# Charrrrrlie/X-as-Supervision

Measured on AMD Instinct MI355X. Metric: images/sec HM36_Multi_SurS1 256px bs32 (full disc+gen training step), higher is better.
Workload: dtype f32 (f16x3 split: every fp32 operand as two fp16 pieces, three products; f32 accumulate); 1 GPU; HM36_Multi_SurS1; batch_per_gpu=32, cameras=4, image=256x256, parallelism=dp1, ranks=1, precision=f16x3, dedupe=False, full=False

## Files before the change

### include/xas_hip.h

```cpp
#ifndef XAS_HIP_H
#define XAS_HIP_H

#include <stddef.h>
#include <stdint.h>

#ifdef __cplusplus
extern "C" {
#endif

const char* xas_last_error(void);
enum {
  XAS_TUNE_WGRAD_SPLIT_XCD = 1,
  XAS_TUNE_PLAIN_KLOOP = 32,
  XAS_TUNE_GLOBAL_LOAD = 64,
  XAS_TUNE_WGRAD_GLOBAL_LOAD = 128,
  XAS_TUNE_WGRAD_ALT_ORDER = 8192,
  XAS_TUNE_WGRAD_PLAIN_KLOOP = 524288,
  XAS_TUNE_SLAB_SHIFT = 15,
  XAS_TUNE_SLAB_MASK = 3,
  XAS_TUNE_SLAB_512 = 32768,
  XAS_TUNE_SLAB_128 = 65536,
  XAS_TUNE_SLAB_64 = 98304,
  XAS_TUNE_COL_REDUCE_LEAN = 262144,
  XAS_TUNE_GENERAL_KERNELS = 1 << 22,
// ... 139 lines not shown
                      const float* var_biased, const float* gamma, const float* beta, float eps, int act,
                      long M, int C, int groups, float* sums, float* workspace,
                      float* dbeta_acc, float* dgamma_acc, const uint8_t* mask, void* stream);
int xas_bn_bwd_apply(const float* x, const float* y, const float* dy, const float* mean,
                     const float* var_biased, const float* gamma, const float* beta, const float* sums,
                     float eps, int act, long M, int C, int groups, double count,
                     float* dx, float* dresidual, const uint8_t* mask, void* stream);
int xas_bn_bwd_apply_amax(const float* x, const float* y, const float* dy, const float* mean,
                          const float* var_biased, const float* gamma, const float* beta, const float* sums,
                          float eps, int act, long M, int C, int groups, double count, float* dx,
                          float* dresidual, const uint8_t* mask, float* amax_out, void* stream);

int xas_maxpool3x3s2_fwd(const float* x, int N, int H, int W, int C, float* y, int8_t* idx, void* stream);
int xas_maxpool3x3s2_bwd(const float* dy, const int8_t* idx, int N, int H, int W, int C, float* dx, void* stream);

int xas_upsample2x_fwd(const float* x, int N, int H, int W, int C, float* y, void* stream);
int xas_upsample2x_bwd(const float* dy, int N, int H, int W, int C, float* dx, void* stream);

int xas_sigmoid_fwd(const float* x, long n, float* y, void* stream);
int xas_sigmoid_bwd(const float* y, const float* dy, long n, float* dx, void* stream);
int xas_nchw_to_nhwc(const float* x, int N, int C, int H, int W, float* y, void* stream);
int xas_nhwc_to_nchw(const float* x, int N, int C, int H, int W, float* y, void* stream);

int xas_warp_affine_u8(const uint8_t* src, const long* src_off, const int* src_hw, const double* minv, int B, int C,
                       int P, uint8_t* dst, void* stream);
int xas_mask_blur_threshold(const uint8_t* mask, int B, int P, uint8_t* out, void* stream);
int xas_patch_finish(const uint8_t* img_bgr, const uint8_t* mask, const float* color_scale, const float* mean3,
                     const float* std3, int rm_bg, int B, int P, float* out_img, float* out_mask, void* stream);
size_t xas_geodesic_workspace_bytes(int B, int P);
int xas_geodesic_weight(const float* mask, const int* centers, const float* params5, int B, int P, float* out,
// ... 73 lines not shown
```

### x-as-supervision_amd/csrc/bn.hip

```cpp
#include "common.h"

namespace xas {


struct ColGeom { int TX, TY, CB, ncb, nslab, G; long rows_per_slab, Mg; };

static int col_geom(long M, int C, int G, ColGeom* g) {
  XAS_REQUIRE(M > 0 && C >= 4 && C % 4 == 0, "column reduce: channel count %d must be a positive multiple of 4", C);
  XAS_REQUIRE(G >= 1 && G <= 64 && M % G == 0, "column reduce: %ld rows do not split into %d equal groups", M, G);
  int cb = 4;
  while (cb < 64 && C % (cb * 2) == 0) cb *= 2;
  g->CB = cb; g->G = G; g->Mg = M / G;
  g->TX = g->CB / 4; g->TY = 256 / g->TX; g->ncb = C / g->CB;
  static const long kWant[4] = {256, 512, 128, 64};
  long want = kWant[(tune_flags() >> XAS_TUNE_SLAB_SHIFT) & XAS_TUNE_SLAB_MASK] * (G > 1 ? 2 : 1) / ((long)g->ncb * G);
  long maxslab = cdiv(g->Mg, (long)g->TY * 8);
  if (want > maxslab) want = maxslab;
  if (want < 1) want = 1;
  g->rows_per_slab = cdiv(g->Mg, want);
  g->nslab = (int)cdiv(g->Mg, g->rows_per_slab);
  return 0;
}

constexpr int kTicketWords = 65536;
// ... 19 lines not shown
  unsafeAtomicAdd(p + 0, v.x); unsafeAtomicAdd(p + 1, v.y); unsafeAtomicAdd(p + 2, v.z); unsafeAtomicAdd(p + 3, v.w);
}

#ifndef XAS_BN_PRIO
#define XAS_BN_PRIO 3
#endif

enum ColMode : int {
  kColStats = 0,
  kColBwdXY = 1,
  kColSum = 2,
  kColBwdY = 3,
  kColBwdX = 4,
  kColStatsPartials = 5,
  kColBwdPartials = 6,
};
constexpr bool col_is_bwd(ColMode m) { return m == kColBwdXY || m == kColBwdY || m == kColBwdX; }
constexpr bool col_two_sums(ColMode m) { return m == kColStats || col_is_bwd(m); }
constexpr bool col_is_stats(ColMode m) { return m == kColStats || m == kColStatsPartials; }

struct ColArgs {
  const float* x; const float* y; const float* dy;
  const float* mean; const float* var;
  const float* gamma; const float* beta;
  const float* pivot;
  const uint8_t* mask;
  float eps; int act; long M; int C; ColGeom g;
  float* partial;
  unsigned* ticket;
  float* out1; float* out2;
  long out_stride;
  float* count_out;
  float* running_mean; float* running_var; float momentum, unbias;
  float* acc1; float* acc2;
  long rows_real;
};

// ... 21 lines not shown
  return dz;
}
__device__ __forceinline__ float4 dz_sign_mask(float4 dz, unsigned mb, float neg) {
  dz.x *= (mb & 1u) ? 1.f : neg; dz.y *= (mb & 2u) ? 1.f : neg; dz.z *= (mb & 4u) ? 1.f : neg; dz.w *= (mb & 8u) ? 1.f : neg;
  return dz;
}
__device__ __forceinline__ float4 xhat4(float4 v, const float4& m, const float4& s) {
  return make_float4((v.x - m.x) * s.x, (v.y - m.y) * s.y, (v.z - m.z) * s.z, (v.w - m.w) * s.w);
}
__device__ __forceinline__ float4 act_inv4(float4 yv, int act) {
  const float up = act == 1 ? 0.f : 100.f;
  return make_float4(yv.x > 0.f ? yv.x : yv.x * up, yv.y > 0.f ? yv.y : yv.y * up, yv.z > 0.f ? yv.z : yv.z * up,
                     yv.w > 0.f ? yv.w : yv.w * up);
}

struct ColChan {
  float4 pivot, mean, rstd, rsg, beta, inv_gamma;
};

template <ColMode MODE>
__device__ __forceinline__ ColChan col_chan(const ColArgs& a, int grp, int c) {
  ColChan ch{};
  if constexpr (MODE == kColStats) ch.pivot = ld4(a.x + (size_t)grp * a.g.Mg * a.C + c);
  if constexpr (MODE == kColBwdXY || MODE == kColBwdX) {
    ch.mean = ld4(a.mean + (size_t)grp * a.C + c);
    const float4 v = ld4(a.var + (size_t)grp * a.C + c);
    ch.rstd = make_float4(rsqrtf(v.x + a.eps), rsqrtf(v.y + a.eps), rsqrtf(v.z + a.eps), rsqrtf(v.w + a.eps));
  }
  if constexpr (MODE == kColBwdX) {
    const float4 gm = ld4(a.gamma + c);
    ch.rsg = make_float4(__fmul_rn(ch.rstd.x, gm.x), __fmul_rn(ch.rstd.y, gm.y), __fmul_rn(ch.rstd.z, gm.z), __fmul_rn(ch.rstd.w, gm.w));
    ch.beta = ld4(a.beta + c);
  }
  if constexpr (MODE == kColBwdY) {
    ch.beta = ld4(a.beta + c);
    const float4 gm = ld4(a.gamma + c);
    ch.inv_gamma = make_float4(gm.x != 0.f ? 1.f / gm.x : 0.f, gm.y != 0.f ? 1.f / gm.y : 0.f, gm.z != 0.f ? 1.f / gm.z : 0.f,
                               gm.w != 0.f ? 1.f / gm.w : 0.f);
  }
  return ch;
}

struct ColTerm { float4 f1, w; };

template <ColMode MODE>
__device__ __forceinline__ ColTerm col_term(const ColArgs& a, const ColChan& ch, long i) {
  const float neg = act_neg_slope(a.act);
  if constexpr (MODE == kColBwdY) {
    const float4 dz = ld4(a.dy + i), yv = ld4(a.y + i);
    return {dz_sign_y(dz, yv, neg), xhat4(act_inv4(yv, a.act), ch.beta, ch.inv_gamma)};
  } else {
    const float4 xv = ld4(a.x + i);
    if constexpr (MODE == kColStats) {
      const float4 d = make_float4(xv.x - ch.pivot.x, xv.y - ch.pivot.y, xv.z - ch.pivot.z, xv.w - ch.pivot.w);
      return {d, d};
    } else if constexpr (MODE == kColBwdXY) {
      float4 dz = ld4(a.dy + i);
      if (a.act && a.mask) dz = dz_sign_mask(dz, a.mask[i >> 2], neg);
      else if (a.act) dz = dz_sign_y(dz, ld4(a.y + i), neg);
      return {dz, xhat4(xv, ch.mean, ch.rstd)};
    } else if constexpr (MODE == kColBwdX) {
      return {dz_sign_x(ld4(a.dy + i), xv, ch.mean, ch.rsg, ch.beta, neg), xhat4(xv, ch.mean, ch.rstd)};
    } else {
      return {xv, xv};
    }
  }
}

__device__ __forceinline__ bool col_publish(const ColArgs& a, float4 (&red)[2][256], __amdgpu_buffer_rsrc_t prs, float4 s1,
                                            float4 s2, int tx, int ty, int c, int grp) {
  const ColGeom& g = a.g;
  red[0][threadIdx.x] = s1; red[1][threadIdx.x] = s2;
  __syncthreads();
  for (int s = g.TY >> 1; s > 0; s >>= 1) {
    if (ty < s) {
      const float4 u0 = red[0][threadIdx.x + s * g.TX], v0 = red[1][threadIdx.x + s * g.TX];
      float4& u = red[0][threadIdx.x]; float4& v = red[1][threadIdx.x];
// ... 87 lines not shown
}

template <ColMode MODE, int UNR, int FL>
__device__ __forceinline__ void col_reduce_body(const ColArgs& a) {
  __shared__ __align__(16) float4 red[2][256];
  const ColGeom& g = a.g;
  const int C = a.C;
  const int tx = threadIdx.x % g.TX, ty = threadIdx.x / g.TX;
  const int c = blockIdx.y * g.CB + tx * 4;
  const int grp = blockIdx.z;
  const long r0 = grp * g.Mg + (long)blockIdx.x * g.rows_per_slab;
  const long r1 = min((grp + 1) * g.Mg, r0 + g.rows_per_slab);
  const ColChan ch = col_chan<MODE>(a, grp, c);
  const float4 z4 = make_float4(0, 0, 0, 0);
  float4 s1 = z4, s2 = z4;
#pragma unroll UNR
  for (long r = r0 + ty; r < r1; r += g.TY) {
    const ColTerm t = col_term<MODE>(a, ch, r * C + c);
    s1.x += t.f1.x; s1.y += t.f1.y; s1.z += t.f1.z; s1.w += t.f1.w;
    if constexpr (col_two_sums(MODE)) {
      s2.x = fmaf(t.f1.x, t.w.x, s2.x); s2.y = fmaf(t.f1.y, t.w.y, s2.y);
      s2.z = fmaf(t.f1.z, t.w.z, s2.z); s2.w = fmaf(t.f1.w, t.w.w, s2.w);
    }
  }
  const __amdgpu_buffer_rsrc_t prs = __builtin_amdgcn_make_buffer_rsrc(
      a.partial, 0, (int)((size_t)g.G * g.nslab * 2 * C * sizeof(float)), 0x00020000);
  if (!col_publish(a, red, prs, s1, s2, tx, ty, c, grp)) return;

  constexpr int L = MODE == kColStatsPartials ? 2 : 4;
  const int cs = MODE == kColStatsPartials ? c >> 1 : c;
  const long n = MODE == kColStatsPartials ? a.rows_real : g.Mg;
  float4 accg1 = z4, accg2 = z4;
  float rm[4] = {0, 0, 0, 0}, rv[4] = {0, 0, 0, 0};
// ... 92 lines not shown
    }
  }
  if (running_mean) { running_mean[c] = rm; running_var[c] = rv; }
}

__device__ __forceinline__ float act_fwd(float v, int act) {
  return act == 0 ? v : (act == 1 ? fmaxf(v, 0.f) : (v > 0.f ? v : 0.01f * v));
}

struct BnChan {
  float4 m, is, rs, g, bt;
  float4 a, b;
};

template <bool BWD>
__device__ __forceinline__ BnChan bn_chan(const float* mean, const float* var, const float* gamma, const float* beta,
                                          const float* sums, float eps, int C4, long i) {
  const int c = (int)(i % C4) * 4;
  BnChan ch;
  const size_t gc = (size_t)blockIdx.y * C4 * 4 + c;
  ch.m = *reinterpret_cast<const float4*>(mean + gc);
  const float4 v = *reinterpret_cast<const float4*>(var + gc);
  ch.g = *reinterpret_cast<const float4*>(gamma + c);
  ch.bt = (!BWD || beta) ? *reinterpret_cast<const float4*>(beta + c) : make_float4(0, 0, 0, 0);
  ch.a = BWD ? *reinterpret_cast<const float4*>(sums + (size_t)blockIdx.y * C4 * 8 + c) : make_float4(0, 0, 0, 0);
  ch.b = BWD ? *reinterpret_cast<const float4*>(sums + (size_t)blockIdx.y * C4 * 8 + (size_t)C4 * 4 + c) : make_float4(0, 0, 0, 0);
  ch.is = make_float4(rsqrtf(v.x + eps), rsqrtf(v.y + eps), rsqrtf(v.z + eps), rsqrtf(v.w + eps));
  ch.rs = make_float4(__fmul_rn(ch.is.x, ch.g.x), __fmul_rn(ch.is.y, ch.g.y), __fmul_rn(ch.is.z, ch.g.z), __fmul_rn(ch.is.w, ch.g.w));
  return ch;
}

template <bool NT> __device__ __forceinline__ void ew_store(float4* p, float4 v) { if (NT) stream_store(p, v); else *p = v; }

__device__ __forceinline__ float4 bn_fwd_elem(const BnChan& ch, float4 xv, float4 rv, int act, bool res, bool has_mask,
                                              uint8_t* mask, float& amx) {
  float4 o;
  o.x = bn_affine(xv.x, ch.m.x, ch.rs.x, ch.bt.x); o.y = bn_affine(xv.y, ch.m.y, ch.rs.y, ch.bt.y);
  o.z = bn_affine(xv.z, ch.m.z, ch.rs.z, ch.bt.z); o.w = bn_affine(xv.w, ch.m.w, ch.rs.w, ch.bt.w);
  if (res) { o.x += rv.x; o.y += rv.y; o.z += rv.z; o.w += rv.w; }
  if (has_mask) *mask = (uint8_t)((o.x > 0.f ? 1u : 0u) | (o.y > 0.f ? 2u : 0u) | (o.z > 0.f ? 4u : 0u) | (o.w > 0.f ? 8u : 0u));
  o.x = act_fwd(o.x, act); o.y = act_fwd(o.y, act); o.z = act_fwd(o.z, act); o.w = act_fwd(o.w, act);
  amx = amax4(amx, o);
  return o;
}

template <bool NT>
__device__ __forceinline__ float4 bn_bwd_elem(const BnChan& ch, float inv_count, float4 xv, float4 yv, float4 dz, unsigned mb,
                                              int act, int sign, bool xh_from_x, bool has_dres, float4* dres, float& amx) {
  const float neg = act_neg_slope(act);
  const float4 &m = ch.m, &is = ch.is, &rs = ch.rs, &g = ch.g, &bt = ch.bt, &a = ch.a, &b = ch.b;
  if (sign == 1) dz = dz_sign_y(dz, yv, neg);
  else if (sign == 2) dz = dz_sign_x(dz, xv, m, rs, bt, neg);
  else if (sign == 3) dz = dz_sign_mask(dz, mb, neg);
  if (has_dres) ew_store<NT>(dres, dz);
  float4 xh;
  if (xh_from_x) xh = xhat4(xv, m, is);
  else {
    const float4 z = act_inv4(yv, act);
    xh.x = g.x != 0.f ? (z.x - bt.x) / g.x : 0.f; xh.y = g.y != 0.f ? (z.y - bt.y) / g.y : 0.f;
    xh.z = g.z != 0.f ? (z.z - bt.z) / g.z : 0.f; xh.w = g.w != 0.f ? (z.w - bt.w) / g.w : 0.f;
  }
  float4 o;
  o.x = g.x * is.x * (dz.x - a.x * inv_count - xh.x * b.x * inv_count);
  o.y = g.y * is.y * (dz.y - a.y * inv_count - xh.y * b.y * inv_count);
  o.z = g.z * is.z * (dz.z - a.z * inv_count - xh.z * b.z * inv_count);
  o.w = g.w * is.w * (dz.w - a.w * inv_count - xh.w * b.w * inv_count);
  amx = fmaxf(fmaxf(amx, fmaxf(fabsf(o.x), fabsf(o.y))), fmaxf(fabsf(o.z), fabsf(o.w)));
  return o;
}

template <bool STREAM, int ACT = 0, bool RES = false, bool MASKOUT = false>
__global__ __launch_bounds__(256) void bn_apply_kernel(const float4* __restrict__ x, const float* __restrict__ mean,
                                                      const float* __restrict__ var, const float* __restrict__ gamma,
                                                      const float* __restrict__ beta, const float4* __restrict__ res,
                                                      float eps, int act_rt, long n4g, int C4, float4* __restrict__ y,
                                                      uint8_t* __restrict__ mask_out, float* __restrict__ amax_out) {
  const int act = STREAM ? ACT : act_rt;
  const bool has_res = STREAM ? RES : res != nullptr, has_mask = STREAM ? MASKOUT : mask_out != nullptr;
  float amx = 0.f;
  if (STREAM) __builtin_amdgcn_s_setprio(XAS_BN_PRIO);
  const long goff = (long)blockIdx.y * n4g;
// ... 101 lines not shown
          const float4 v = *reinterpret_cast<const float4*>(xn + ((size_t)hi * W + wi) * C + c);
          const int tap = r * 3 + s;
          if (first || v.x > best.x) { best.x = v.x; b0 = tap; }
          if (first || v.y > best.y) { best.y = v.y; b1 = tap; }
          if (first || v.z > best.z) { best.z = v.z; b2 = tap; }
          if (first || v.w > best.w) { best.w = v.w; b3 = tap; }
          first = false;
        }
      }
      *reinterpret_cast<float4*>(y + (obase + e) * 4) = best;
      *reinterpret_cast<char4*>(idx + (obase + e) * 4) = make_char4((char)b0, (char)b1, (char)b2, (char)b3);
    }
  }
}

__global__ __launch_bounds__(256) void maxpool_bwd_kernel(const float* __restrict__ dy, const int8_t* __restrict__ idx, int N, int H,
                                                          int W, int C, int Ho, int Wo, float* __restrict__ dx) {
  const int C4 = C / 4, per_row = W * C4;
  for (int row = blockIdx.x; row < N * H; row += gridDim.x) {
    const int n = row / H, hi = row - n * H;
    const size_t obase = (size_t)row * per_row;
    for (int e = threadIdx.x; e < per_row; e += blockDim.x) {
      const int wi = e / C4, c = (e - wi * C4) * 4;
      float4 acc = make_float4(0, 0, 0, 0);
      for (int ho = hi / 2; ho <= (hi + 1) / 2; ++ho) {
        if (ho >= Ho) continue;
        const int r = hi - (ho * 2 - 1);
        if (r < 0 || r > 2) continue;
        for (int wo = wi / 2; wo <= (wi + 1) / 2; ++wo) {
          if (wo >= Wo) continue;
          const int s = wi - (wo * 2 - 1);
          if (s < 0 || s > 2) continue;
          const size_t o = (((size_t)n * Ho + ho) * Wo + wo) * C + c;
          const char4 k = *reinterpret_cast<const char4*>(idx + o);
          const float4 g = *reinterpret_cast<const float4*>(dy + o);
          const int tap = r * 3 + s;
          if (k.x == tap) acc.x += g.x;
          if (k.y == tap) acc.y += g.y;
          if (k.z == tap) acc.z += g.z;
          if (k.w == tap) acc.w += g.w;
        }
      }
      stream_store(reinterpret_cast<float4*>(dx) + obase + e, acc);
    }
  }
}

__device__ __forceinline__ unsigned xcd_contiguous(unsigned b, unsigned nblk) {
  const unsigned per = (nblk + 7u) >> 3;
  return (b & 7u) * per + (b >> 3);
}

__global__ __launch_bounds__(256) void upsample2x_fwd_kernel(const float* __restrict__ x, int N, int H, int W, int C,
                                                             float* __restrict__ y, unsigned segs, unsigned nblk) {
  const unsigned C4 = (unsigned)C / 4, Ho = 2u * H, Wo = 2u * W;
  const unsigned bid = xcd_contiguous(blockIdx.x, nblk);
  if (bid >= nblk) return;
  const unsigned row = bid / segs, seg = bid - row * segs;
  const unsigned n = row / Ho, ho = row - n * Ho;
  const unsigned e = seg * 256u + threadIdx.x;
// ... 366 lines not shown
  return 0;
}

extern "C" int xas_maxpool3x3s2_bwd(const float* dy, const int8_t* idx, int N, int H, int W, int C, float* dx,
                                    void* stream) {
  XAS_REQUIRE(dy && dx && idx && N > 0 && H > 0 && W > 0 && C % 4 == 0, "maxpool bwd: bad arguments");
  const int Ho = (H + 2 - 3) / 2 + 1, Wo = (W + 2 - 3) / 2 + 1;
  XAS_REQUIRE((long)N * H < 0x7fffffffl, "maxpool bwd: too many rows");
  const long rows = (long)N * H;
  hipLaunchKernelGGL(maxpool_bwd_kernel, dim3((unsigned)(rows < 16384 ? rows : 16384)), dim3(256), 0, as_stream(stream), dy, idx, N, H,
                     W, C, Ho, Wo, dx);
  XAS_LAUNCH_CHECK();
  return 0;
}

extern "C" int xas_upsample2x_fwd(const float* x, int N, int H, int W, int C, float* y, void* stream) {
  XAS_REQUIRE(x && y && N > 0 && H > 0 && W > 0 && C % 4 == 0, "upsample2x: bad arguments");
  const long segs = cdiv((long)2 * W * (C / 4), 256), blocks = (long)N * 2 * H * segs;
  XAS_REQUIRE(blocks < 0x7ffffff0l && (long)N * 4 * H * W * C < (1l << 40), "upsample2x: tensor too large");
  hipLaunchKernelGGL(upsample2x_fwd_kernel, dim3((unsigned)(8 * cdiv(blocks, 8))), dim3(256), 0, as_stream(stream), x, N, H,
                     W, C, y, (unsigned)segs, (unsigned)blocks);
  XAS_LAUNCH_CHECK();
  return 0;
}

extern "C" int xas_upsample2x_bwd(const float* dy, int N, int H, int W, int C, float* dx, void* stream) {
  XAS_REQUIRE(dy && dx && N > 0 && H > 0 && W > 0 && C % 4 == 0, "upsample2x bwd: bad arguments");
  const long segs = cdiv((long)W * (C / 4), 256), blocks = (long)N * H * segs;
  XAS_REQUIRE(blocks < 0x7ffffff0l && (long)N * 4 * H * W * C < (1l << 40), "upsample2x bwd: tensor too large");
  hipLaunchKernelGGL(upsample2x_bwd_kernel, dim3((unsigned)(8 * cdiv(blocks, 8))), dim3(256), 0, as_stream(stream), dy, N,
// ... 35 lines not shown
```

### x-as-supervision_amd/modules/integral_base_modules/resnet.py

```python
import torch.nn as nn

from xas_amd import layers as L
import os

from xas_amd.ops_nn import ACT_NONE, ACT_RELU, bottleneck, from_nchw

FUSED_BLOCKS = os.environ.get('XAS_FUSED_BLOCKS', '1') == '1'


class Bottleneck(nn.Module):
    expansion = 4

    def __init__(self, inplanes, planes, stride=1, downsample=None):
        super().__init__()
        k = 'kaiming_fan_out'
        self.conv1 = L.Conv2d(inplanes, planes, 1, bias=False, init=k)
        self.bn1 = L.BatchNorm2d(planes, act=ACT_RELU)
        self.conv2 = L.Conv2d(planes, planes, 3, stride=stride, padding=1, bias=False, init=k)
        self.bn2 = L.BatchNorm2d(planes, act=ACT_RELU)
        self.conv3 = L.Conv2d(planes, planes * 4, 1, bias=False, init=k)
        self.bn3 = L.BatchNorm2d(planes * 4, act=ACT_RELU)
        self.downsample = downsample
        self.stride = stride
        self._fused_params = None
# ... 46 lines not shown
        self.layer3 = self._stage(block, 256, layers[2], 2)
        self.layer4 = self._stage(block, 512, layers[3], 2)

    def _stage(self, block, planes, count, stride):
        proj = None
        if stride != 1 or self.inplanes != planes * block.expansion:
            proj = nn.Sequential(
                L.Conv2d(self.inplanes, planes * block.expansion, 1, stride=stride, bias=False, init='kaiming_fan_out'),
                L.BatchNorm2d(planes * block.expansion, act=ACT_NONE, sync=True))
        blocks = [block(self.inplanes, planes, stride, proj)]
        self.inplanes = planes * block.expansion
        blocks += [block(self.inplanes, planes) for _ in range(1, count)]
        return nn.Sequential(*blocks)

    def forward(self, x):
        x = self.maxpool(self.bn1(self.conv1(from_nchw(x))))
        return self.layer4(self.layer3(self.layer2(self.layer1(x))))
```

### x-as-supervision_amd/xas_amd/_lib.py

```python
import ctypes
import os

import torch

_HERE = os.path.dirname(os.path.abspath(__file__))
LIB_PATH = os.environ.get('XAS_HIP_LIB') or os.path.join(_HERE, 'libxas_hip.so')
_lib = None
ABI_VERSION = 3

_T = {'p': ctypes.c_void_p, 'i': ctypes.c_int, 'l': ctypes.c_long, 'f': ctypes.c_float, 'u': ctypes.c_uint,
      'd': ctypes.c_double, 'z': ctypes.c_size_t}


class ConvShape(ctypes.Structure):
    _fields_ = [(n, ctypes.c_int) for n in ('N', 'Hi', 'Wi', 'Cin', 'Cout', 'R', 'S', 'stride', 'pad', 'Ho', 'Wo', 'mode')] + [
        ('grad_amax', ctypes.c_void_p),
        ('x_amax', ctypes.c_void_p)]


PREC_F32, PREC_BF16, PREC_BF16X6, PREC_F16X3 = 0, 1, 2, 3
PREC_NAMES = {'f32': PREC_F32, 'bf16': PREC_BF16, 'bf16x6': PREC_BF16X6, 'f16x3': PREC_F16X3}

GUARD_FLOATS = 8
GUARD_NORM, GUARD_SCALE, GUARD_SKIP, GUARD_T, GUARD_SKIPPED, GUARD_STEP_SIZE, GUARD_INV_SQRT_BC2, GUARD_NONFINITE = range(8)
# ... 53 lines not shown
    'xas_bn_stats': ('pliipplppppflp', 'i'),
    'xas_bn_stats_from_partials': ('pliilppplppppfp', 'i'),
    'xas_bn_bwd_sums_from_partials': ('pliippppp', 'i'),
    'xas_bn_sync_merge': ('piiilppppfp', 'i'),
    'xas_col_sum': ('plippp', 'i'),
    'xas_col_sum_acc': ('plippp', 'i'),
    'xas_bn_apply': ('ppppppfiliippp', 'i'),
    'xas_bn_apply_amax': ('ppppppfiliipppp', 'i'),
    'xas_abs_max': ('plpp', 'i'),
    'xas_bn_update_running': ('ppppfliip', 'i'),
    'xas_bn_bwd_reduce': ('pppppppfiliipppppp', 'i'),
    'xas_bn_bwd_apply': ('ppppppppfiliidpppp', 'i'),
    'xas_bn_bwd_apply_amax': ('ppppppppfiliidppppp', 'i'),
    'xas_maxpool3x3s2_fwd': ('piiiippp', 'i'),
    'xas_maxpool3x3s2_bwd': ('ppiiiipp', 'i'),
    'xas_upsample2x_fwd': ('piiiipp', 'i'),
    'xas_upsample2x_bwd': ('piiiipp', 'i'),
    'xas_sigmoid_fwd': ('plpp', 'i'),
    'xas_sigmoid_bwd': ('pplpp', 'i'),
    'xas_nchw_to_nhwc': ('piiiipp', 'i'),
    'xas_nhwc_to_nchw': ('piiiipp', 'i'),
    'xas_warp_affine_u8': ('ppppiiipp', 'i'),
    'xas_mask_blur_threshold': ('piipp', 'i'),
    'xas_patch_finish': ('pppppiiippp', 'i'),
    'xas_geodesic_workspace_bytes': ('ii', 'z'),
    'xas_geodesic_weight': ('pppiipppp', 'i'),
    'xas_geodesic_weight_multi': ('ppiipiipppp', 'i'),
    'xas_loss_nblk': ('l', 'i'),
    'xas_mask_loss_fwd': ('pppliPpp'.replace('P', 'p'), 'i'),
    'xas_mask_loss_bwd': ('pppliPppp'.replace('P', 'p'), 'i'),
# ... 93 lines not shown
```

### x-as-supervision_amd/xas_amd/ops_nn.py

```python
import os

import torch
import torch.distributed as dist

from . import _lib
from . import streams
from ._lib import ConvShape, call, ptr, query

CL = torch.channels_last
_weights_epoch = [0]

_groups = [1]

_prefix = [0, 0]


class bn_groups:
    def __init__(self, groups, prefix_groups=0, images_per_group=0):
        self.groups = int(groups)
        self.prefix = [int(prefix_groups) * int(images_per_group), int(prefix_groups)]
        if self.prefix[1] and not (0 < self.prefix[1] < self.groups and images_per_group > 0):
            raise RuntimeError('bn_groups: the no-grad prefix must be a proper, non-empty subset of the groups')

    def __enter__(self):
# ... 795 lines not shown

def _sync_stats(mean, var, count, group):
    world = dist.get_world_size(group)
    C = mean.numel()
    packed = torch.cat([mean, var, mean.new_tensor([float(count)])])
    gathered = torch.empty(world * (2 * C + 1), device=mean.device, dtype=torch.float32)
    dist.all_gather_into_tensor(gathered, packed, group=group)
    g = gathered.view(world, 2 * C + 1).double()
    cnt = g[:, 2 * C:]
    total = cnt.sum()
    gm = (g[:, :C] * cnt).sum(0) / total
    gv = ((g[:, C:2 * C] + (g[:, :C] - gm) ** 2) * cnt).sum(0) / total
    return gm.float().contiguous(), gv.float().contiguous()


def _bn_forward(x, gamma, beta, running_mean, running_var, residual, training, momentum, eps, act, group, stats_fn=None):
    x_tail = to_cl(x)
    x = _full(x_tail)
    if x is not x_tail and not training:
        raise RuntimeError('prefix pass: training-mode norms only')
    n, c, h, w = x.shape
    G = _groups[0]
    if n % G:
        raise RuntimeError('batch of %d images does not split into %d camera groups' % (n, G))
    M = n * h * w
    Mg = M // G
    dev = x.device
    count = float(Mg)
    if training:
        if stats_fn is None:
            ws = torch.empty(query('xas_bn_workspace_floats', M, c, G), device=dev, dtype=torch.float32)

            def stats_fn(mean_p, var_p, out_stride, count_p, rm_p, rv_p, mom):
                call('xas_bn_stats', ptr(x), M, c, G, mean_p, var_p, out_stride, count_p, ptr(ws), rm_p, rv_p, float(mom), int(Mg))
        if group is None:
# ... 26 lines not shown
                book, cur = streams.book_stream(), torch.cuda.current_stream()
                book.wait_stream(cur)
                with torch.cuda.stream(book):
                    call('xas_bn_update_running', ptr(mean), ptr(var), ptr(running_mean), ptr(running_var),
                         float(momentum), int(count), c, G)
                mean.record_stream(book)
                var.record_stream(book)
            else:
                call('xas_bn_sync_merge', ptr(gathered), world, G, c, stride, ptr(mean), ptr(var),
                     ptr(running_mean), ptr(running_var), float(momentum))
        if bn_log['on'] and running_mean is not None:
            bn_log['calls'].append((mean, var, running_mean, running_var, momentum, count, G))
    else:
        mean = running_mean.reshape(1, c).expand(G, c).contiguous() if G > 1 else running_mean
        var = running_var.reshape(1, c).expand(G, c).contiguous() if G > 1 else running_var
    res = _full(to_cl(residual)) if residual is not None else None
    y = torch.empty_like(x)
    masked = training and residual is not None and act != ACT_NONE and os.environ.get('XAS_BN_MASK', '1') == '1'
    mask = torch.empty(M * c // 4, device=dev, dtype=torch.uint8) if masked else None
    slot = grad_amax_slot(dev) if x.is_cuda else None
    call('xas_bn_apply_amax', ptr(x), ptr(mean), ptr(var), ptr(gamma), ptr(beta), ptr(res), float(eps), act, M, c, G, ptr(y), ptr(mask),
         ptr(slot))
    if slot is not None:
        tag_grad_amax(y, slot)
    xfree = training and act == ACT_LEAKY and residual is None
    yfree = training and act == ACT_RELU and residual is None and os.environ.get('XAS_BN_YFREE', '1') == '1'
    if x is not x_tail:
        k = _prefix[1]
        y = _tail(y)
        if slot is not None:
# ... 98 lines not shown
        ctx.shape = (n, c, h, w)
        return y

    @staticmethod
    def backward(ctx, dy):
        (idx,) = ctx.saved_tensors
        n, c, h, w = ctx.shape
        dy = to_cl(dy)
        dx = empty_cl(n, c, h, w, dy)
        call('xas_maxpool3x3s2_bwd', ptr(dy), ptr(idx), n, h, w, c, ptr(dx))
        return dx


def maxpool3x3s2(x):
    return _MaxPool.apply(x)


class _Upsample2x(torch.autograd.Function):
    @staticmethod
    def forward(ctx, x):
        if _prefix[0]:
            raise RuntimeError('prefix pass: up-sampling is not on the detector path')
        x = to_cl(x)
        n, c, h, w = x.shape
        y = empty_cl(n, c, 2 * h, 2 * w, x)
        call('xas_upsample2x_fwd', ptr(x), n, h, w, c, ptr(y))
        pass_amax(y, x)
        ctx.shape = (n, c, h, w)
        return y

# ... 135 lines not shown
```

### x-as-supervision_amd/xas_amd/prof.py

```python
import torch

from . import _lib

CONV_ENTRIES = ('xas_conv_fwd', 'xas_conv_fwd_head', 'xas_conv_fwd_bnstats', 'xas_conv_dgrad', 'xas_conv_dgrad_acc', 'xas_conv_dgrad_acc_masked', 'xas_conv_wgrad',
                'xas_conv_wgrad_oihw', 'xas_conv_wgrad_acc')


BN_ENTRIES = ('xas_bn_stats', 'xas_bn_apply', 'xas_bn_apply_amax', 'xas_bn_bwd_reduce', 'xas_bn_bwd_apply', 'xas_bn_bwd_apply_amax')


def bn_bytes(name, a):
    if name == 'xas_bn_stats':
        return 4.0 * a[1] * a[2]
    if name in ('xas_bn_apply', 'xas_bn_apply_amax'):
        t = 4.0 * a[8] * a[9]
        return t * (2 + (1 if a[5] else 0)) + (t / 16 if a[12] else 0.0)
    if name == 'xas_bn_bwd_reduce':
        t = 4.0 * a[9] * a[10]
        return t * (1 + (1 if a[0] else 0) + (1 if a[1] else 0)) + (t / 16 if a[16] else 0.0)
    t = 4.0 * a[10] * a[11]
    return t * (2 + (1 if a[0] else 0) + (1 if a[1] else 0) + (1 if a[15] else 0)) + (t / 16 if a[16] else 0.0)


def conv_flops(shape):
    return 2.0 * shape.N * shape.Ho * shape.Wo * shape.Cout * shape.R * shape.S * shape.Cin


def conv_bytes(shape):
    return 4.0 * (shape.N * shape.Hi * shape.Wi * shape.Cin + shape.Cout * shape.R * shape.S * shape.Cin
                  + shape.N * shape.Ho * shape.Wo * shape.Cout)

# ... 67 lines not shown
```

Before: 2072 images/s.

## Fuse stem batchnorm+ReLU with 3x3 maxpool in forward and backward

Adds fused kernels that apply the stem batch norm and ReLU while computing the 3x3 stride-2 max pool, so the full-resolution normalized activation is never written. In backward, the pooled gradient is scattered on the fly inside the BN reduce and apply passes instead of being materialized by a separate maxpool backward. This removes several full-size activation reads and writes at the largest spatial resolution. In exchange, each 3x3 window recomputes the normalization per tap and gathers up to four pooled gradients per input pixel, which adds compute and index arithmetic.

```diff
diff --git a/include/xas_hip.h b/include/xas_hip.h
--- a/include/xas_hip.h
+++ b/include/xas_hip.h
@@ -177,6 +177,18 @@
 int xas_maxpool3x3s2_fwd(const float* x, int N, int H, int W, int C, float* y, int8_t* idx, void* stream);
 int xas_maxpool3x3s2_bwd(const float* dy, const int8_t* idx, int N, int H, int W, int C, float* dx, void* stream);
 
+int xas_bn_apply_maxpool_amax(const float* x, const float* mean, const float* var_biased, const float* gamma,
+                              const float* beta, float eps, int act, int N, int H, int W, int C, int groups,
+                              float* y_pooled, int8_t* idx, float* amax_out, void* stream);
+int xas_bn_bwd_reduce_pooled(const float* x, const float* dy_pooled, const int8_t* idx, const float* mean,
+                             const float* var_biased, const float* gamma, const float* beta, float eps, int act,
+                             int N, int H, int W, int C, int groups, float* sums, float* workspace,
+                             float* dbeta_acc, float* dgamma_acc, void* stream);
+int xas_bn_bwd_apply_pooled_amax(const float* x, const float* dy_pooled, const int8_t* idx, const float* mean,
+                                 const float* var_biased, const float* gamma, const float* beta, const float* sums,
+                                 float eps, int act, int N, int H, int W, int C, int groups, double count, float* dx,
+                                 float* amax_out, void* stream);
+
 int xas_upsample2x_fwd(const float* x, int N, int H, int W, int C, float* y, void* stream);
 int xas_upsample2x_bwd(const float* dy, int N, int H, int W, int C, float* dx, void* stream);
 
diff --git a/x-as-supervision_amd/csrc/bn.hip b/x-as-supervision_amd/csrc/bn.hip
--- a/x-as-supervision_amd/csrc/bn.hip
+++ b/x-as-supervision_amd/csrc/bn.hip
@@ -57,13 +57,16 @@
   kColBwdX = 4,
   kColStatsPartials = 5,
   kColBwdPartials = 6,
+  kColBwdXPooled = 7,
 };
-constexpr bool col_is_bwd(ColMode m) { return m == kColBwdXY || m == kColBwdY || m == kColBwdX; }
+constexpr bool col_sign_from_x(ColMode m) { return m == kColBwdX || m == kColBwdXPooled; }
+constexpr bool col_is_bwd(ColMode m) { return m == kColBwdXY || m == kColBwdY || col_sign_from_x(m); }
 constexpr bool col_two_sums(ColMode m) { return m == kColStats || col_is_bwd(m); }
 constexpr bool col_is_stats(ColMode m) { return m == kColStats || m == kColStatsPartials; }
 
 struct ColArgs {
   const float* x; const float* y; const float* dy;
+  const int8_t* pool_idx; int H, W, Ho, Wo;
   const float* mean; const float* var;
   const float* gamma; const float* beta;
   const float* pivot;
@@ -115,6 +118,29 @@
                      yv.w > 0.f ? yv.w : yv.w * up);
 }
 
+__device__ __forceinline__ float4 maxpool_grad_at(const float* __restrict__ dy, const int8_t* __restrict__ idx, int n, int hi,
+                                                  int wi, int c, int Ho, int Wo, int C);
+
+struct ColPix { int n, hi, wi, dn, dh, dw; };
+__device__ __forceinline__ ColPix col_pix(const ColArgs& a, long r, int stride) {
+  const int hw = a.H * a.W;
+  ColPix p;
+  p.n = (int)(r / hw);
+  const int rem = (int)(r - (long)p.n * hw);
+  p.hi = rem / a.W; p.wi = rem - p.hi * a.W;
+  p.dn = stride / hw;
+  const int srem = stride - p.dn * hw;
+  p.dh = srem / a.W; p.dw = srem - p.dh * a.W;
+  return p;
+}
+__device__ __forceinline__ void col_pix_next(const ColArgs& a, ColPix& p) {
+  p.wi += p.dw;
+  if (p.wi >= a.W) { p.wi -= a.W; ++p.hi; }
+  p.hi += p.dh;
+  if (p.hi >= a.H) { p.hi -= a.H; ++p.n; }
+  p.n += p.dn;
+}
+
 struct ColChan {
   float4 pivot, mean, rstd, rsg, beta, inv_gamma;
 };
@@ -123,12 +149,12 @@
 __device__ __forceinline__ ColChan col_chan(const ColArgs& a, int grp, int c) {
   ColChan ch{};
   if constexpr (MODE == kColStats) ch.pivot = ld4(a.x + (size_t)grp * a.g.Mg * a.C + c);
-  if constexpr (MODE == kColBwdXY || MODE == kColBwdX) {
+  if constexpr (MODE == kColBwdXY || col_sign_from_x(MODE)) {
     ch.mean = ld4(a.mean + (size_t)grp * a.C + c);
     const float4 v = ld4(a.var + (size_t)grp * a.C + c);
     ch.rstd = make_float4(rsqrtf(v.x + a.eps), rsqrtf(v.y + a.eps), rsqrtf(v.z + a.eps), rsqrtf(v.w + a.eps));
   }
-  if constexpr (MODE == kColBwdX) {
+  if constexpr (col_sign_from_x(MODE)) {
     const float4 gm = ld4(a.gamma + c);
     ch.rsg = make_float4(__fmul_rn(ch.rstd.x, gm.x), __fmul_rn(ch.rstd.y, gm.y), __fmul_rn(ch.rstd.z, gm.z), __fmul_rn(ch.rstd.w, gm.w));
     ch.beta = ld4(a.beta + c);
@@ -145,8 +171,9 @@
 struct ColTerm { float4 f1, w; };
 
 template <ColMode MODE>
-__device__ __forceinline__ ColTerm col_term(const ColArgs& a, const ColChan& ch, long i) {
+__device__ __forceinline__ ColTerm col_term(const ColArgs& a, const ColChan& ch, long r, int c, const ColPix& px) {
   const float neg = act_neg_slope(a.act);
+  const long i = r * a.C + c;
   if constexpr (MODE == kColBwdY) {
     const float4 dz = ld4(a.dy + i), yv = ld4(a.y + i);
     return {dz_sign_y(dz, yv, neg), xhat4(act_inv4(yv, a.act), ch.beta, ch.inv_gamma)};
@@ -162,6 +189,9 @@
       return {dz, xhat4(xv, ch.mean, ch.rstd)};
     } else if constexpr (MODE == kColBwdX) {
       return {dz_sign_x(ld4(a.dy + i), xv, ch.mean, ch.rsg, ch.beta, neg), xhat4(xv, ch.mean, ch.rstd)};
+    } else if constexpr (MODE == kColBwdXPooled) {
+      const float4 dy = maxpool_grad_at(a.dy, a.pool_idx, px.n, px.hi, px.wi, c, a.Ho, a.Wo, a.C);
+      return {dz_sign_x(dy, xv, ch.mean, ch.rsg, ch.beta, neg), xhat4(xv, ch.mean, ch.rstd)};
     } else {
       return {xv, xv};
     }
@@ -279,9 +309,12 @@
   const ColChan ch = col_chan<MODE>(a, grp, c);
   const float4 z4 = make_float4(0, 0, 0, 0);
   float4 s1 = z4, s2 = z4;
+  ColPix px{};
+  if constexpr (MODE == kColBwdXPooled) px = col_pix(a, r0 + ty, g.TY);
 #pragma unroll UNR
   for (long r = r0 + ty; r < r1; r += g.TY) {
-    const ColTerm t = col_term<MODE>(a, ch, r * C + c);
+    const ColTerm t = col_term<MODE>(a, ch, r, c, px);
+    if constexpr (MODE == kColBwdXPooled) col_pix_next(a, px);
     s1.x += t.f1.x; s1.y += t.f1.y; s1.z += t.f1.z; s1.w += t.f1.w;
     if constexpr (col_two_sums(MODE)) {
       s2.x = fmaf(t.f1.x, t.w.x, s2.x); s2.y = fmaf(t.f1.y, t.w.y, s2.y);
@@ -404,20 +437,24 @@
 };
 
 template <bool BWD>
-__device__ __forceinline__ BnChan bn_chan(const float* mean, const float* var, const float* gamma, const float* beta,
-                                          const float* sums, float eps, int C4, long i) {
-  const int c = (int)(i % C4) * 4;
+__device__ __forceinline__ BnChan bn_chan_at(const float* mean, const float* var, const float* gamma, const float* beta,
+                                             const float* sums, float eps, int C4, int grp, int c) {
   BnChan ch;
-  const size_t gc = (size_t)blockIdx.y * C4 * 4 + c;
+  const size_t gc = (size_t)grp * C4 * 4 + c;
   ch.m = *reinterpret_cast<const float4*>(mean + gc);
   const float4 v = *reinterpret_cast<const float4*>(var + gc);
   ch.g = *reinterpret_cast<const float4*>(gamma + c);
   ch.bt = (!BWD || beta) ? *reinterpret_cast<const float4*>(beta + c) : make_float4(0, 0, 0, 0);
-  ch.a = BWD ? *reinterpret_cast<const float4*>(sums + (size_t)blockIdx.y * C4 * 8 + c) : make_float4(0, 0, 0, 0);
-  ch.b = BWD ? *reinterpret_cast<const float4*>(sums + (size_t)blockIdx.y * C4 * 8 + (size_t)C4 * 4 + c) : make_float4(0, 0, 0, 0);
+  ch.a = BWD ? *reinterpret_cast<const float4*>(sums + (size_t)grp * C4 * 8 + c) : make_float4(0, 0, 0, 0);
+  ch.b = BWD ? *reinterpret_cast<const float4*>(sums + (size_t)grp * C4 * 8 + (size_t)C4 * 4 + c) : make_float4(0, 0, 0, 0);
   ch.is = make_float4(rsqrtf(v.x + eps), rsqrtf(v.y + eps), rsqrtf(v.z + eps), rsqrtf(v.w + eps));
   ch.rs = make_float4(__fmul_rn(ch.is.x, ch.g.x), __fmul_rn(ch.is.y, ch.g.y), __fmul_rn(ch.is.z, ch.g.z), __fmul_rn(ch.is.w, ch.g.w));
   return ch;
+}
+template <bool BWD>
+__device__ __forceinline__ BnChan bn_chan(const float* mean, const float* var, const float* gamma, const float* beta,
+                                          const float* sums, float eps, int C4, long i) {
+  return bn_chan_at<BWD>(mean, var, gamma, beta, sums, eps, C4, blockIdx.y, (int)(i % C4) * 4);
 }
 
 template <bool NT> __device__ __forceinline__ void ew_store(float4* p, float4 v) { if (NT) stream_store(p, v); else *p = v; }
@@ -434,7 +471,14 @@
   return o;
 }
 
-template <bool NT>
+template <int FORM>
+__device__ __forceinline__ float bn_dx_lane(float g, float is, float dz, float a, float b, float xh, float inv_count) {
+  if constexpr (FORM == 0) return g * is * (dz - a * inv_count - xh * b * inv_count);
+  const float t = FORM == 1 ? __fsub_rn(dz, __fmul_rn(a, inv_count)) : __fmaf_rn(-inv_count, a, dz);
+  return __fmul_rn(__fmul_rn(g, is), __fmaf_rn(-inv_count, __fmul_rn(xh, b), t));
+}
+
+template <bool NT, int FORM = 0>
 __device__ __forceinline__ float4 bn_bwd_elem(const BnChan& ch, float inv_count, float4 xv, float4 yv, float4 dz, unsigned mb,
                                               int act, int sign, bool xh_from_x, bool has_dres, float4* dres, float& amx) {
   const float neg = act_neg_slope(act);
@@ -451,10 +495,10 @@
     xh.z = g.z != 0.f ? (z.z - bt.z) / g.z : 0.f; xh.w = g.w != 0.f ? (z.w - bt.w) / g.w : 0.f;
   }
   float4 o;
-  o.x = g.x * is.x * (dz.x - a.x * inv_count - xh.x * b.x * inv_count);
-  o.y = g.y * is.y * (dz.y - a.y * inv_count - xh.y * b.y * inv_count);
-  o.z = g.z * is.z * (dz.z - a.z * inv_count - xh.z * b.z * inv_count);
-  o.w = g.w * is.w * (dz.w - a.w * inv_count - xh.w * b.w * inv_count);
+  o.x = bn_dx_lane<FORM>(g.x, is.x, dz.x, a.x, b.x, xh.x, inv_count);
+  o.y = bn_dx_lane<FORM>(g.y, is.y, dz.y, a.y, b.y, xh.y, inv_count);
+  o.z = bn_dx_lane<FORM>(g.z, is.z, dz.z, a.z, b.z, xh.z, inv_count);
+  o.w = bn_dx_lane<FORM>(g.w, is.w, dz.w, a.w, b.w, xh.w, inv_count);
   amx = fmaxf(fmaxf(amx, fmaxf(fabsf(o.x), fabsf(o.y))), fmaxf(fabsf(o.z), fabsf(o.w)));
   return o;
 }
@@ -586,6 +630,30 @@
   }
 }
 
+__device__ __forceinline__ float4 maxpool_grad_at(const float* __restrict__ dy, const int8_t* __restrict__ idx, int n, int hi,
+                                                  int wi, int c, int Ho, int Wo, int C) {
+  const int ho0 = hi >> 1, wo0 = wi >> 1;
+  const bool h1 = (hi & 1) && ho0 + 1 < Ho, w1 = (wi & 1) && wo0 + 1 < Wo;
+  const int t0 = ((hi & 1) + 1) * 3, s0 = (wi & 1) + 1;
+  const size_t o = (((size_t)n * Ho + ho0) * Wo + wo0) * C + c, dh = h1 ? (size_t)Wo * C : 0, dw = w1 ? (size_t)C : 0;
+  const size_t off[4] = {o, o + dw, o + dh, o + dh + dw};
+  const int tap[4] = {t0 + s0, t0, s0, 0};
+  const bool on[4] = {true, w1, h1, h1 && w1};
+  char4 k[4];
+  float4 g[4];
+#pragma unroll
+  for (int j = 0; j < 4; ++j) { k[j] = *reinterpret_cast<const char4*>(idx + off[j]); g[j] = *reinterpret_cast<const float4*>(dy + off[j]); }
+  float4 acc = make_float4(0, 0, 0, 0);
+#pragma unroll
+  for (int j = 0; j < 4; ++j) {
+    acc.x += on[j] && k[j].x == tap[j] ? g[j].x : 0.f;
+    acc.y += on[j] && k[j].y == tap[j] ? g[j].y : 0.f;
+    acc.z += on[j] && k[j].z == tap[j] ? g[j].z : 0.f;
+    acc.w += on[j] && k[j].w == tap[j] ? g[j].w : 0.f;
+  }
+  return acc;
+}
+
 __global__ __launch_bounds__(256) void maxpool_bwd_kernel(const float* __restrict__ dy, const int8_t* __restrict__ idx, int N, int H,
                                                           int W, int C, int Ho, int Wo, float* __restrict__ dx) {
   const int C4 = C / 4, per_row = W * C4;
@@ -594,28 +662,84 @@
     const size_t obase = (size_t)row * per_row;
     for (int e = threadIdx.x; e < per_row; e += blockDim.x) {
       const int wi = e / C4, c = (e - wi * C4) * 4;
-      float4 acc = make_float4(0, 0, 0, 0);
-      for (int ho = hi / 2; ho <= (hi + 1) / 2; ++ho) {
-        if (ho >= Ho) continue;
-        const int r = hi - (ho * 2 - 1);
-        if (r < 0 || r > 2) continue;
-        for (int wo = wi / 2; wo <= (wi + 1) / 2; ++wo) {
-          if (wo >= Wo) continue;
-          const int s = wi - (wo * 2 - 1);
-          if (s < 0 || s > 2) continue;
-          const size_t o = (((size_t)n * Ho + ho) * Wo + wo) * C + c;
-          const char4 k = *reinterpret_cast<const char4*>(idx + o);
-          const float4 g = *reinterpret_cast<const float4*>(dy + o);
+      stream_store(reinterpret_cast<float4*>(dx) + obase + e, maxpool_grad_at(dy, idx, n, hi, wi, c, Ho, Wo, C));
+    }
+  }
+}
+
+template <bool KEEP>
+__global__ __launch_bounds__(256) void bn_apply_maxpool_kernel(const float* __restrict__ x, const float* __restrict__ mean,
+                                                              const float* __restrict__ var, const float* __restrict__ gamma,
+                                                              const float* __restrict__ beta, float eps, int N, int H, int W,
+                                                              int C, int Ho, int Wo, int npg, float* __restrict__ y,
+                                                              int8_t* __restrict__ idx, float* __restrict__ amax_out) {
+  __builtin_amdgcn_s_setprio(XAS_BN_PRIO);
+  const int C4 = C / 4, per_row = Wo * C4;
+  const float4 z4 = make_float4(0, 0, 0, 0);
+  float amx = 0.f, tap_amx = 0.f;
+  for (int row = blockIdx.x; row < N * Ho; row += gridDim.x) {
+    const int n = row / Ho, ho = row - n * Ho;
+    const float* xn = x + (size_t)n * H * W * C;
+    const size_t obase = (size_t)row * per_row;
+    BnChan ch;
+    if (KEEP) ch = bn_chan_at<false>(mean, var, gamma, beta, nullptr, eps, C4, n / npg, (int)(threadIdx.x % C4) * 4);
+    for (int e = threadIdx.x; e < per_row; e += blockDim.x) {
+      const int wo = e / C4, c = (e - wo * C4) * 4;
+      if (!KEEP) ch = bn_chan_at<false>(mean, var, gamma, beta, nullptr, eps, C4, n / npg, c);
+      float4 best = make_float4(-INFINITY, -INFINITY, -INFINITY, -INFINITY);
+      int b0 = 0, b1 = 0, b2 = 0, b3 = 0;
+      bool first = true;
+#pragma unroll
+      for (int r = 0; r < 3; ++r) {
+        const int hi = ho * 2 - 1 + r;
+        if ((unsigned)hi >= (unsigned)H) continue;
+#pragma unroll
+        for (int s = 0; s < 3; ++s) {
+          const int wi = wo * 2 - 1 + s;
+          if ((unsigned)wi >= (unsigned)W) continue;
+          const float4 xv = *reinterpret_cast<const float4*>(xn + ((size_t)hi * W + wi) * C + c);
+          const float4 v = bn_fwd_elem(ch, xv, z4, 1, false, false, nullptr, tap_amx);
           const int tap = r * 3 + s;
-          if (k.x == tap) acc.x += g.x;
-          if (k.y == tap) acc.y += g.y;
-          if (k.z == tap) acc.z += g.z;
-          if (k.w == tap) acc.w += g.w;
+          if (first || v.x > best.x) { best.x = v.x; b0 = tap; }
+          if (first || v.y > best.y) { best.y = v.y; b1 = tap; }
+          if (first || v.z > best.z) { best.z = v.z; b2 = tap; }
+          if (first || v.w > best.w) { best.w = v.w; b3 = tap; }
+          first = false;
         }
       }
-      stream_store(reinterpret_cast<float4*>(dx) + obase + e, acc);
-    }
-  }
+      amx = amax4(amx, best);
+      stream_store(reinterpret_cast<float4*>(y) + obase + e, best);
+      __builtin_nontemporal_store(b0 | b1 << 8 | b2 << 16 | b3 << 24, reinterpret_cast<int*>(idx) + obase + e);
+    }
+  }
+  if (amax_out) publish_amax(amax_out, amx);
+}
+
+template <bool KEEP>
+__global__ __launch_bounds__(256) void bn_bwd_apply_pooled_kernel(
+    const float* __restrict__ x, const float* __restrict__ dy, const int8_t* __restrict__ idx, const float* __restrict__ mean,
+    const float* __restrict__ var, const float* __restrict__ gamma, const float* __restrict__ beta,
+    const float* __restrict__ sums, float eps, int N, int H, int W, int C, int Ho, int Wo, int npg, float inv_count,
+    float* __restrict__ dx, float* __restrict__ amax_out) {
+  __builtin_amdgcn_s_setprio(XAS_BN_PRIO);
+  const int C4 = C / 4, per_row = W * C4;
+  const float4 z4 = make_float4(0, 0, 0, 0);
+  float amx = 0.f;
+  for (int row = blockIdx.x; row < N * H; row += gridDim.x) {
+    const int n = row / H, hi = row - n * H;
+    const size_t obase = (size_t)row * per_row;
+    BnChan ch;
+    if (KEEP) ch = bn_chan_at<true>(mean, var, gamma, beta, sums, eps, C4, n / npg, (int)(threadIdx.x % C4) * 4);
+    for (int e = threadIdx.x; e < per_row; e += blockDim.x) {
+      const int wi = e / C4, c = (e - wi * C4) * 4;
+      if (!KEEP) ch = bn_chan_at<true>(mean, var, gamma, beta, sums, eps, C4, n / npg, c);
+      const float4 xv = stream_load(reinterpret_cast<const float4*>(x) + obase + e);
+      const float4 dz = maxpool_grad_at(dy, idx, n, hi, wi, c, Ho, Wo, C);
+      stream_store(reinterpret_cast<float4*>(dx) + obase + e,
+                   bn_bwd_elem<true, KEEP ? 1 : 2>(ch, inv_count, xv, z4, dz, 0u, 1, 2, true, false, nullptr, amx));
+    }
+  }
+  if (amax_out) publish_amax(amax_out, amx);
 }
 
 __device__ __forceinline__ unsigned xcd_contiguous(unsigned b, unsigned nblk) {
@@ -1012,6 +1136,65 @@
   return 0;
 }
 
+static int pooled_geom(const char* who, int act, int N, int H, int W, int C, int groups, int* Ho, int* Wo, int* npg) {
+  XAS_REQUIRE(act == 1, "%s: the fused norm + pool passes are for ReLU (act 1), got act %d", who, act);
+  XAS_REQUIRE(N > 0 && H > 0 && W > 0 && C >= 4 && C % 4 == 0 && groups >= 1 && N % groups == 0,
+              "%s: bad shape N=%d H=%d W=%d C=%d (a multiple of 4) groups=%d", who, N, H, W, C, groups);
+  XAS_REQUIRE((long)N * H < 0x7fffffffl && (long)H * W < 0x7fffffffl, "%s: too many rows", who);
+  *Ho = (H + 2 - 3) / 2 + 1; *Wo = (W + 2 - 3) / 2 + 1; *npg = N / groups;
+  return 0;
+}
+
+extern "C" int xas_bn_apply_maxpool_amax(const float* x, const float* mean, const float* var_biased, const float* gamma,
+                                         const float* beta, float eps, int act, int N, int H, int W, int C, int groups,
+                                         float* y_pooled, int8_t* idx, float* amax_out, void* stream) {
+  int Ho, Wo, npg;
+  if (pooled_geom("bn_apply_maxpool", act, N, H, W, C, groups, &Ho, &Wo, &npg)) return 1;
+  XAS_REQUIRE(x && mean && var_biased && gamma && beta && y_pooled && idx, "bn_apply_maxpool: null buffer");
+  const long rows = (long)N * Ho;
+  hipLaunchKernelGGL(256 % (C / 4) == 0 ? bn_apply_maxpool_kernel<true> : bn_apply_maxpool_kernel<false>, dim3((unsigned)(rows < 8192 ? rows : 8192)), dim3(256), 0, as_stream(stream), x, mean,
+                     var_biased, gamma, beta, eps, N, H, W, C, Ho, Wo, npg, y_pooled, idx, amax_out);
+  XAS_LAUNCH_CHECK();
+  return 0;
+}
+
+extern "C" int xas_bn_bwd_reduce_pooled(const float* x, const float* dy_pooled, const int8_t* idx, const float* mean,
+                                        const float* var_biased, const float* gamma, const float* beta, float eps, int act,
+                                        int N, int H, int W, int C, int groups, float* sums, float* workspace,
+                                        float* dbeta_acc, float* dgamma_acc, void* stream) {
+  int Ho, Wo, npg;
+  if (pooled_geom("bn_bwd_reduce_pooled", act, N, H, W, C, groups, &Ho, &Wo, &npg)) return 1;
+  const long M = (long)N * H * W;
+  ColGeom g;
+  if (col_geom(M, C, groups, &g)) return 1;
+  XAS_REQUIRE(x && dy_pooled && idx && mean && var_biased && gamma && beta && sums && workspace, "bn_bwd_reduce_pooled: null buffer");
+  XAS_REQUIRE((dbeta_acc == nullptr) == (dgamma_acc == nullptr), "bn_bwd_reduce_pooled: gradient accumulators come in pairs");
+  const bool lean = (tune_flags() & XAS_TUNE_COL_REDUCE_LEAN) != 0;
+  ColArgs a{};
+  if (col_args(&a, g, M, C, workspace)) return 1;
+  a.x = x; a.dy = dy_pooled; a.pool_idx = idx; a.H = H; a.W = W; a.Ho = Ho; a.Wo = Wo;
+  a.mean = mean; a.var = var_biased; a.gamma = gamma; a.beta = beta; a.eps = eps; a.act = act;
+  a.out1 = sums; a.out2 = sums + C; a.out_stride = 2 * (long)C;
+  a.acc1 = dbeta_acc; a.acc2 = dgamma_acc;
+  return launch_col_reduce<kColBwdXPooled>(a, lean, stream);
+}
+
+extern "C" int xas_bn_bwd_apply_pooled_amax(const float* x, const float* dy_pooled, const int8_t* idx, const float* mean,
+                                            const float* var_biased, const float* gamma, const float* beta, const float* sums,
+                                            float eps, int act, int N, int H, int W, int C, int groups, double count, float* dx,
+                                            float* amax_out, void* stream) {
+  int Ho, Wo, npg;
+  if (pooled_geom("bn_bwd_apply_pooled", act, N, H, W, C, groups, &Ho, &Wo, &npg)) return 1;
+  XAS_REQUIRE(x && dy_pooled && idx && mean && var_biased && gamma && beta && sums && dx && count > 0,
+              "bn_bwd_apply_pooled: null buffer / bad count");
+  const long rows = (long)N * H;
+  hipLaunchKernelGGL(256 % (C / 4) == 0 ? bn_bwd_apply_pooled_kernel<true> : bn_bwd_apply_pooled_kernel<false>, dim3((unsigned)(rows < 16384 ? rows : 16384)), dim3(256), 0, as_stream(stream), x,
+                     dy_pooled, idx, mean, var_biased, gamma, beta, sums, eps, N, H, W, C, Ho, Wo, npg, (float)(1.0 / count), dx,
+                     amax_out);
+  XAS_LAUNCH_CHECK();
+  return 0;
+}
+
 extern "C" int xas_upsample2x_fwd(const float* x, int N, int H, int W, int C, float* y, void* stream) {
   XAS_REQUIRE(x && y && N > 0 && H > 0 && W > 0 && C % 4 == 0, "upsample2x: bad arguments");
   const long segs = cdiv((long)2 * W * (C / 4), 256), blocks = (long)N * 2 * H * segs;
diff --git a/x-as-supervision_amd/modules/integral_base_modules/resnet.py b/x-as-supervision_amd/modules/integral_base_modules/resnet.py
--- a/x-as-supervision_amd/modules/integral_base_modules/resnet.py
+++ b/x-as-supervision_amd/modules/integral_base_modules/resnet.py
@@ -3,7 +3,7 @@
 from xas_amd import layers as L
 import os
 
-from xas_amd.ops_nn import ACT_NONE, ACT_RELU, bottleneck, from_nchw
+from xas_amd.ops_nn import ACT_NONE, ACT_RELU, bottleneck, from_nchw, norm_relu_pool, norm_relu_pool_fusable
 
 FUSED_BLOCKS = os.environ.get('XAS_FUSED_BLOCKS', '1') == '1'
 
@@ -84,5 +84,12 @@
         return nn.Sequential(*blocks)
 
     def forward(self, x):
-        x = self.maxpool(self.bn1(self.conv1(from_nchw(x))))
+        x = self.conv1(from_nchw(x))
+        bn = self.bn1
+        if norm_relu_pool_fusable(bn.training, bn.act, x.shape[1], x):
+            group = bn.sync_group()
+            bn.count_batch()
+            x = norm_relu_pool(x, bn.weight, bn.bias, bn.running_mean, bn.running_var, bn.momentum, bn.eps, group)
+        else:
+            x = self.maxpool(bn(x))
         return self.layer4(self.layer3(self.layer2(self.layer1(x))))
diff --git a/x-as-supervision_amd/xas_amd/_lib.py b/x-as-supervision_amd/xas_amd/_lib.py
--- a/x-as-supervision_amd/xas_amd/_lib.py
+++ b/x-as-supervision_amd/xas_amd/_lib.py
@@ -91,6 +91,9 @@
     'xas_bn_bwd_apply_amax': ('ppppppppfiliidppppp', 'i'),
     'xas_maxpool3x3s2_fwd': ('piiiippp', 'i'),
     'xas_maxpool3x3s2_bwd': ('ppiiiipp', 'i'),
+    'xas_bn_apply_maxpool_amax': ('pppppfiiiiiipppp', 'i'),
+    'xas_bn_bwd_reduce_pooled': ('pppppppfiiiiiippppp', 'i'),
+    'xas_bn_bwd_apply_pooled_amax': ('ppppppppfiiiiiidppp', 'i'),
     'xas_upsample2x_fwd': ('piiiipp', 'i'),
     'xas_upsample2x_bwd': ('piiiipp', 'i'),
     'xas_sigmoid_fwd': ('plpp', 'i'),
diff --git a/x-as-supervision_amd/xas_amd/ops_nn.py b/x-as-supervision_amd/xas_amd/ops_nn.py
--- a/x-as-supervision_amd/xas_amd/ops_nn.py
+++ b/x-as-supervision_amd/xas_amd/ops_nn.py
@@ -833,11 +833,7 @@
     return gm.float().contiguous(), gv.float().contiguous()
 
 
-def _bn_forward(x, gamma, beta, running_mean, running_var, residual, training, momentum, eps, act, group, stats_fn=None):
-    x_tail = to_cl(x)
-    x = _full(x_tail)
-    if x is not x_tail and not training:
-        raise RuntimeError('prefix pass: training-mode norms only')
+def _bn_statistics(x, running_mean, running_var, training, momentum, group, stats_fn=None):
     n, c, h, w = x.shape
     G = _groups[0]
     if n % G:
@@ -894,6 +890,19 @@
     else:
         mean = running_mean.reshape(1, c).expand(G, c).contiguous() if G > 1 else running_mean
         var = running_var.reshape(1, c).expand(G, c).contiguous() if G > 1 else running_var
+    return mean, var, count
+
+
+def _bn_forward(x, gamma, beta, running_mean, running_var, residual, training, momentum, eps, act, group, stats_fn=None):
+    x_tail = to_cl(x)
+    x = _full(x_tail)
+    if x is not x_tail and not training:
+        raise RuntimeError('prefix pass: training-mode norms only')
+    n, c, h, w = x.shape
+    G = _groups[0]
+    M = n * h * w
+    dev = x.device
+    mean, var, count = _bn_statistics(x, running_mean, running_var, training, momentum, group, stats_fn)
     res = _full(to_cl(residual)) if residual is not None else None
     y = torch.empty_like(x)
     masked = training and residual is not None and act != ACT_NONE and os.environ.get('XAS_BN_MASK', '1') == '1'
@@ -1022,6 +1031,78 @@
 
 def maxpool3x3s2(x):
     return _MaxPool.apply(x)
+
+
+STEM_FUSE = os.environ.get('XAS_STEM_FUSE', '1') == '1'
+
+
+class _NormReluPool(torch.autograd.Function):
+
+    @staticmethod
+    def forward(ctx, x, gamma, beta, running_mean, running_var, momentum, eps, group):
+        x_tail = to_cl(x)
+        x = _full(x_tail)
+        n, c, h, w = x.shape
+        G = _groups[0]
+        mean, var, count = _bn_statistics(x, running_mean, running_var, True, momentum, group)
+        ho, wo = (h - 1) // 2 + 1, (w - 1) // 2 + 1
+        yf = empty_cl(n, c, ho, wo, x)
+        idxf = torch.empty(n * ho * wo * c, device=x.device, dtype=torch.int8)
+        slot = grad_amax_slot(x.device)
+        call('xas_bn_apply_maxpool_amax', ptr(x), ptr(mean), ptr(var), ptr(gamma), ptr(beta), float(eps), ACT_RELU, n, h, w, c, G,
+             ptr(yf), ptr(idxf), ptr(slot))
+        y, idx = _tail(yf), _tail(idxf, per_image=ho * wo * c)
+        if slot is not None:
+            tag_grad_amax(y, slot)
+        if x is not x_tail:
+            k = _prefix[1]
+            n, G = n - _prefix[0], G - k
+            mean, var = mean[k:], var[k:]
+            x = x_tail
+        ctx.save_for_backward(x, idx, mean, var, gamma, beta)
+        ctx.cfg = (n, c, h, w, G, float(eps), count, group)
+        if ctx.needs_input_grad[1] and ctx.needs_input_grad[2]:
+            note_use(gamma)
+            note_use(beta)
+        return y
+
+    @staticmethod
+    def backward(ctx, dy):
+        x, idx, mean, var, gamma, beta = ctx.saved_tensors
+        n, c, h, w, G, eps, count, group = ctx.cfg
+        dy = to_cl(dy)
+        dev = x.device
+        sums = torch.empty(G, 2, c, device=dev, dtype=torch.float32)
+        ws = torch.empty(query('xas_bn_workspace_floats', n * h * w, c, G), device=dev, dtype=torch.float32)
+        gg, gb = gamma.grad, beta.grad
+        direct = (ctx.needs_input_grad[1] and ctx.needs_input_grad[2] and gg is not None and gb is not None
+                  and gg.is_contiguous() and gb.is_contiguous() and gg.dtype == torch.float32 and gb.dtype == torch.float32)
+        call('xas_bn_bwd_reduce_pooled', ptr(x), ptr(dy), ptr(idx), ptr(mean), ptr(var), ptr(gamma), ptr(beta), eps, ACT_RELU,
+             n, h, w, c, G, ptr(sums), ptr(ws), ptr(gb) if direct else None, ptr(gg) if direct else None)
+        if direct:
+            dgamma = dbeta = None
+            grad_ready(gamma)
+            grad_ready(beta)
+        else:
+            dgamma, dbeta = sums[:, 1].sum(0), sums[:, 0].sum(0)
+        if group is not None:
+            from . import dp as _dp
+            _dp.timed_collective(lambda: dist.all_reduce(sums, group=group), sums.numel() * 4)
+        dx = torch.empty_like(x)
+        slot = grad_amax_slot(dev)
+        call('xas_bn_bwd_apply_pooled_amax', ptr(x), ptr(dy), ptr(idx), ptr(mean), ptr(var), ptr(gamma), ptr(beta), ptr(sums),
+             eps, ACT_RELU, n, h, w, c, G, float(count), ptr(dx), ptr(slot))
+        if slot is not None:
+            tag_grad_amax(dx, slot)
+        return dx, dgamma, dbeta, None, None, None, None, None
+
+
+def norm_relu_pool_fusable(training, act, c, x):
+    return STEM_FUSE and training and act == ACT_RELU and c % 4 == 0 and x.is_cuda
+
+
+def norm_relu_pool(x, gamma, beta, running_mean, running_var, momentum=0.1, eps=1e-5, group=None):
+    return _NormReluPool.apply(x, gamma, beta, running_mean, running_var, momentum, eps, group)
 
 
 class _Upsample2x(torch.autograd.Function):
diff --git a/x-as-supervision_amd/xas_amd/prof.py b/x-as-supervision_amd/xas_amd/prof.py
--- a/x-as-supervision_amd/xas_amd/prof.py
+++ b/x-as-supervision_amd/xas_amd/prof.py
@@ -6,7 +6,8 @@
                 'xas_conv_wgrad_oihw', 'xas_conv_wgrad_acc')
 
 
-BN_ENTRIES = ('xas_bn_stats', 'xas_bn_apply', 'xas_bn_apply_amax', 'xas_bn_bwd_reduce', 'xas_bn_bwd_apply', 'xas_bn_bwd_apply_amax')
+BN_ENTRIES = ('xas_bn_stats', 'xas_bn_apply', 'xas_bn_apply_amax', 'xas_bn_bwd_reduce', 'xas_bn_bwd_apply', 'xas_bn_bwd_apply_amax',
+              'xas_bn_apply_maxpool_amax', 'xas_bn_bwd_reduce_pooled', 'xas_bn_bwd_apply_pooled_amax')
 
 
 def bn_bytes(name, a):
@@ -15,6 +16,11 @@
     if name in ('xas_bn_apply', 'xas_bn_apply_amax'):
         t = 4.0 * a[8] * a[9]
         return t * (2 + (1 if a[5] else 0)) + (t / 16 if a[12] else 0.0)
+    if name in ('xas_bn_apply_maxpool_amax', 'xas_bn_bwd_reduce_pooled', 'xas_bn_bwd_apply_pooled_amax'):
+        n, h, w, c = a[7:11] if name == 'xas_bn_apply_maxpool_amax' else (a[9:13] if name == 'xas_bn_bwd_reduce_pooled' else a[10:14])
+        t = 4.0 * n * h * w * c
+        p = 1.25 * 4.0 * n * ((h - 1) // 2 + 1) * ((w - 1) // 2 + 1) * c
+        return t + p + (t if name == 'xas_bn_bwd_apply_pooled_amax' else 0.0)
     if name == 'xas_bn_bwd_reduce':
         t = 4.0 * a[9] * a[10]
         return t * (1 + (1 if a[0] else 0) + (1 if a[1] else 0)) + (t / 16 if a[16] else 0.0)
```

New measurement: 2087 images/s (median of 6 runs). About the same (+0.7%).
